# willow-ahrens/ChainPartitioners.jl

Hardware: AMD Instinct MI355X
Metric: partitions/sec, DynamicTotalSplitter(AffineConnectivityModel{Int64}(0,0,0,1)), K=64 (higher is better)
Workload: dtype int64; 1 GPU; config 3: DynamicTotalSplitter(AffineConnectivityModel{Int64}(0,0,0,1)) on suitesparse_shaped CSR (seeded SplitMix64 generator, tests/synth.py), n=10000000 rows, nnz=100000000, K=64; one independent partition per GPU; n=10000000, nnz=100000000, K=64, includes_oracle_build=True, device_block_pool=True

## Files before the change

chainpartitioners.jl_amd/csrc/capi.hip:

```cpp
#include "csr.hpp"
#include "model.hpp"
#include "dp.hpp"
#include "weight.hpp"
#include "sym.hpp"
#include "cut.hpp"
#include <cmath>
#include <memory>

using namespace cpk;

namespace cpk {

__global__ void __launch_bounds__(256) k_range_counts(int64_t nq, const int64_t *__restrict__ P, const int64_t *__restrict__ Rr,
                                                      const int64_t *__restrict__ pos, const int32_t *__restrict__ prev,
                                                      const int64_t *__restrict__ fpos, const int32_t *__restrict__ flast,
                                                      unsigned long long *__restrict__ nets, unsigned long long *__restrict__ selfnets)
{
    int64_t i = blockIdx.x;
    if (i >= nq) return;
    __shared__ int64_t sh[256];
    int64_t p = P[i], r = Rr[i];
    int64_t stride = (int64_t)gridDim.y * 256, start = (int64_t)blockIdx.y * 256 + threadIdx.x;
    int64_t c = 0;
    if (r > p) {
// ... 96 lines not shown

template <typename TC>
static int32_t oracle_eval_into(cp_csr_t A, const cp_model_t *model, const cp_rowpart_t *Pi, int64_t nq, const int64_t *j, const int64_t *jp,
                                const int64_t *k, TC *out)
{
    const bool i64 = std::is_same<TC, int64_t>::value;
    return cp_oracle_eval(A, model, Pi, CP_HINT_STEP, nq, j, jp, k, i64 ? (int64_t *)out : nullptr, i64 ? nullptr : (double *)out);
}

static const struct { const char *name; int64_t *var; bool kept; } g_stats[] = {
    {"spec_redo", &g_spec_redo, false}, {"poison_hits", &g_poison_hits, false}, {"fix_trips", &g_fix_trips, false},
    {"fix_edges", &g_fix_edges, false}, {"fix_items", &g_fix_items, false}, {"bn_sym_layers", &g_bn_sym_layers, true},
    {"own_split_tiles", &g_own_split_tiles, false}, {"gap_split_tiles", &g_gap_split_tiles, false},
    {"own_pair_waves", &g_own_pair_waves, false}, {"own_pair_lone", &g_own_pair_lone, false},
    {"overlap_isect", &g_overlap_isect, false}, {"cut_scan_layers", &g_cut_scan_layers, false},
};
static void stats_reset(bool all) { for (const auto &c : g_stats) if (all || !c.kept) *c.var = 0; }

enum OptRule { OPT_PLAIN, OPT_BOOL, OPT_CLAMP, OPT_POW2 };
constexpr int64_t NOLIM_LO = INT64_MIN, NOLIM_HI = INT64_MAX;
static const struct Opt { const char *name; int64_t *var; OptRule rule; int64_t lo, hi; } g_options[] = {
    {"force_brute", &g_opt_force_brute, OPT_PLAIN, 0, 0}, {"brute_max_n", &g_opt_brute_max_n, OPT_PLAIN, 0, 0}, {"dbg", &g_opt_dbg, OPT_PLAIN, 0, 0},
    {"short_t", &g_opt_short_t, OPT_PLAIN, 0, 0}, {"short_e", &g_opt_short_e, OPT_PLAIN, 0, 0}, {"ra_cache", &g_opt_ra_cache, OPT_PLAIN, 0, 0},
    {"leaf", &g_opt_leaf, OPT_PLAIN, 0, 0}, {"block_tables", &g_opt_block_tables, OPT_PLAIN, 0, 0}, {"nospec", &g_opt_nospec, OPT_PLAIN, 0, 0},
    {"rpass_small_tau", &g_opt_rpass_small_tau, OPT_PLAIN, 0, 0}, {"fixed_point", &g_opt_fixed_point, OPT_PLAIN, 0, 0},
    {"bn_wave", &g_opt_bn_wave, OPT_PLAIN, 0, 0},
    {"poison", &g_opt_poison, OPT_PLAIN, 0, 0},
    {"pool", &g_opt_pool, OPT_BOOL, 0, 0},
    {"own_blk", &g_opt_own_blk, OPT_BOOL, 0, 0},
    {"own_split", &g_opt_own_split, OPT_BOOL, 0, 0},
    {"own_pair", &g_opt_own_pair, OPT_BOOL, 0, 0},
    {"gap_split", &g_opt_gap_split, OPT_BOOL, 0, 0},
    {"lws", &g_opt_lws, OPT_BOOL, 0, 0},
    {"gap_tau", &g_opt_gap_tau, OPT_CLAMP, NOLIM_LO, 20}, {"gap_min", &g_opt_gap_min, OPT_CLAMP, 8, NOLIM_HI}, {"gap_nr", &g_opt_gap_nr, OPT_CLAMP, 1, 2},
    {"force_max", &g_opt_force_max, OPT_CLAMP, 0, NOLIM_HI}, {"rpass_cap", &g_opt_rpass_cap, OPT_CLAMP, 1, NOLIM_HI},
    {"own_min", &g_opt_own_min, OPT_CLAMP, 64, NOLIM_HI}, {"bn_chunk", &g_opt_bn_chunk, OPT_CLAMP, 1, NOLIM_HI},
    {"bn_slack", &g_opt_bn_slack, OPT_CLAMP, 0, NOLIM_HI}, {"bn_run", &g_opt_bn_run, OPT_CLAMP, 2, NOLIM_HI},
    {"rpass_ch", &g_opt_rpass_ch, OPT_POW2, 16, 4096}, {"setup_bs", &g_opt_setup_bs, OPT_POW2, 64, 1024}, {"lws_leaf", &g_opt_lws_leaf, OPT_POW2, 256, 2048},
};
static int64_t opt_value(const Opt &o, int64_t value)
{
    switch (o.rule) {
    case OPT_BOOL: return value ? 1 : 0;
    case OPT_CLAMP: return value < o.lo ? o.lo : value > o.hi ? o.hi : value;
    case OPT_POW2: { int64_t v = o.lo; while (v < value && v < o.hi) v <<= 1; return v; }
    default: return value;
    }
}

// ... 586 lines not shown
```

chainpartitioners.jl_amd/csrc/dp.hpp:

```cpp
#pragma once
#include "csr.hpp"
#include "model.hpp"

struct cp_dp_s {
    cp_csr_s *A = nullptr;
    int64_t K = 0;
    int32_t combine = 0, order = 0;
    bool fast = false, fast_bn = false, need_self = false;
    void *work = nullptr;
    cpk::DBuf<int32_t> ptr;
    int64_t rlo = 0, rhi = 0;
    int64_t wwin = 0;
    std::vector<int64_t> lay_lo, lay_hi;
    virtual ~cp_dp_s() = default;
    virtual int32_t step_layer(int64_t k, const void *cst_prev_device, void *cst_cur_device) = 0;
    virtual int32_t block_tables(int32_t *nplanes_out, int64_t *opt_out, int64_t *nets_out, int64_t *selfnets_out) = 0;
};

namespace cpk {

using DpBase = ::cp_dp_s;

struct DpWindow {
    int64_t w = 0;
// ... 84 lines not shown
extern int64_t g_opt_ra_cache;
extern int64_t g_opt_fixed_point;
extern int64_t g_opt_nospec;
extern int64_t g_spec_redo;
extern int64_t g_opt_rpass_small_tau;
extern int64_t g_opt_force_max;
extern int64_t g_opt_setup_bs;
extern int64_t g_opt_rpass_cap;
extern int64_t g_opt_rpass_ch;
extern int64_t g_opt_own_min;
extern int64_t g_opt_own_blk;
extern int64_t g_opt_own_split;
extern int64_t g_own_split_tiles;
extern int64_t g_opt_gap_split;
extern int64_t g_gap_split_tiles;
extern int64_t g_opt_own_pair;
extern int64_t g_own_pair_waves, g_own_pair_lone;
void dp_own_pair_test(int64_t nt, int64_t wave, int64_t *res);
extern int64_t g_overlap_isect;
void dp_own_split_test(cp_csr_s *A, int32_t *vpos_out, int32_t *vsa_out, int32_t *vnext_out, int64_t *res);
extern int64_t g_opt_short_t, g_opt_short_e;
extern int64_t g_opt_force_brute;
extern int64_t g_opt_brute_max_n;
extern int64_t g_opt_dbg;
enum DbgBit : int64_t {
    DBG_PRINT_ROUNDS = 8,
    DBG_NO_INTERIOR = 32,
    DBG_NO_OWN_TILES = 64,
    DBG_POISON = 128,
    DBG_POISON_ZERO = 256,
// ... 17 lines not shown
```

chainpartitioners.jl_amd/csrc/dp_brute.hip:

```cpp
#include "csr.hpp"
#include "model.hpp"
#include "dp.hpp"

namespace cpk {

int64_t g_opt_force_brute = 0;
int64_t g_opt_short_t = 8, g_opt_short_e = 64;
int64_t g_opt_own_min = 64;
int64_t g_opt_own_blk = 1;
int64_t g_opt_own_split = 1;
int64_t g_own_split_tiles = 0;
int64_t g_opt_gap_split = 1;
int64_t g_gap_split_tiles = 0;
int64_t g_opt_own_pair = 1;
int64_t g_own_pair_waves = 0, g_own_pair_lone = 0;
int64_t g_opt_rpass_ch = 256;
int64_t g_opt_rpass_small_tau = 4;
int64_t g_opt_force_max = 1024;
int64_t g_opt_setup_bs = 1024;
int64_t g_opt_rpass_cap = 200;
int64_t g_opt_nospec = 0, g_spec_redo = 0;
int64_t g_opt_gap_tau = 6, g_opt_gap_min = 64, g_opt_gap_nr = 2;
int64_t g_opt_ra_cache = 1;
int64_t g_opt_leaf = 1, g_opt_block_tables = 0;
int64_t g_opt_poison = 0, g_poison_hits = 0;
int64_t g_fix_trips = 0, g_fix_edges = 0, g_fix_items = 0;
int64_t g_opt_fixed_point = 0;
int64_t g_opt_brute_max_n = 200000;
int64_t g_opt_dbg = 0;

// ... 63 lines not shown
```

chainpartitioners.jl_amd/csrc/dp_total.hip:

```cpp
#include "dp_total.hpp"
#include <optional>

namespace cpk {

struct RoundDesc {
    int32_t isA, tau, nbits, nextra;
    Geo G;
    int64_t aoff[32];
    int64_t n, ntask;
    int64_t tbase[36];
    int64_t tskip[36];
    int64_t a_r0, a_nmain;
    int64_t extra[64];
    int32_t nlast, last_b[31];
    int32_t skip_std, skip_mir;
    int32_t fin_stamp;
};

__device__ __forceinline__ void decode_task(const RoundDesc &R, int64_t t, int64_t &r, int &b)
{
    if (R.G.win) {
        int bb = R.isA ? 0 : R.tau + 1;
        while (t >= R.tbase[bb + 1]) bb++;
        const int64_t l = t - R.tbase[bb] + R.tskip[bb];
// ... 1103 lines not shown
        for (int j = 0; j < 4; j++) {
            int32_t q = base + 64 * j + lane;
            fl[j] = false;
            if (q < e1) { int32_t v = arr[q]; fl[j] = GE ? (v >= thr) : (v < thr); }
        }
#pragma unroll
        for (int j = 0; j < 4; j++) {
            unsigned long long m = __ballot(fl[j]);
            int32_t w = myend - (base + 64 * j);
            if (w > 0) mine += __popcll(w >= 64 ? m : (m & ((1ull << w) - 1ull)));
        }
    }
    return c + mine;
}

template <typename TC, bool HYP>
struct GapCtx {
    const Best<TC, HYP> *part, *sub; const int32_t *spv; const uint8_t *spec;
    const int64_t *tilePS, *tilePS2;
    const int32_t *pos, *next, *fpos, *flast;
    const TC *W;
    int blk;
};

template <typename TC, bool HYP, int NR, bool SLOW>
__device__ __forceinline__ bool gap_walk(const GapCtx<TC, HYP> &C, const DevModel<TC> &M, TC alpha, int64_t ka, int64_t kz, int64_t k0,
                                         int32_t B, int32_t L, int32_t r, int32_t posr, const int32_t (&rr)[NR], const int32_t (&rcmp)[NR],
                                         const bool (&valid)[NR], int lane,
                                         TC (&bv)[NR], int32_t (&bp)[NR], int32_t (&bl)[NR], int32_t (&bl2)[NR], int32_t (&cum)[NR], int32_t (&cum2)[NR])
{
    const int64_t ps0 = C.tilePS[k0], ps20 = HYP ? C.tilePS2[k0] : 0;
    for (int64_t kb = ka; kb < kz; kb += 64) {
    const int64_t km = kb + lane < kz ? kb + lane : kz - 1;
    const int32_t m_base = (int32_t)(C.tilePS[km] - ps0), m_base2 = HYP ? (int32_t)(C.tilePS2[km] - ps20) : 0;
    const int m_ns = C.spec[km];
    Best<TC, HYP> m_part; best_clear(m_part);
    if (m_ns == 0) m_part = C.part[km];
    const int nb = (int)(kz - kb < 64 ? kz - kb : 64);
    Best<TC, HYP> nx_c; best_clear(nx_c);
    int32_t nx_sv = 0;
    {
        const int ns0 = rdl(m_ns, 0);
        if (ns0 > 0 && ns0 <= SMAX) { if (lane <= ns0) nx_c = C.sub[kb * (SMAX + 1) + lane]; if (lane < ns0) nx_sv = C.spv[kb * (SMAX + 1) + lane]; }
    }
    for (int i = 0; i < nb; i++) {
        const int64_t k = kb + i;
        const int32_t base = rdl(m_base, i), base2 = HYP ? rdl(m_base2, i) : 0;
        const int ns = rdl(m_ns, i);
        const Best<TC, HYP> cur_c = nx_c;
        const int32_t cur_sv = nx_sv;
        if (i + 1 < nb) {
            const int ns1 = rdl(m_ns, i + 1);
// ... 96 lines not shown
    g.rL = r - (1 << tau);
    int64_t hi64 = (int64_t)r + ((int64_t)1 << tau), re = ((((int64_t)r >> b) + 1) << b);
    if (hi64 > re) hi64 = re;
    if (hi64 > n + 1) hi64 = n + 1;
    g.hi = (int32_t)hi64;
    g.rr = g.rL + 1 + 64 * ck + lane;
    g.none = g.rL + 1 + 64 * ck >= g.hi;
    g.valid = g.rr < g.hi;
    g.rcmp = g.valid ? g.rr : INT32_MAX;
    return g;
}

template <typename TC, bool HYP>
struct GapSegRec { TC v; int32_t p, l, l2, cum, cum2, _pad; };

template <typename TC, bool HYP, int NR, bool SLOW>
__global__ void __launch_bounds__(256, 4) k_gap_finish(int tau, int nchunk, RoundCounts *__restrict__ rc, int64_t n,
                                                    const int64_t *__restrict__ toffs, GapCtx<TC, HYP> C,
                                                    const int4 *__restrict__ tdesc, const uint8_t *__restrict__ tb, const int32_t *__restrict__ rlen,
                                                    const int32_t *__restrict__ prev, const int32_t *__restrict__ lpos, const int32_t *__restrict__ lfirst,
                                                    DevModel<TC> M, TC alpha,
                                                    int32_t *__restrict__ opt, int32_t *__restrict__ nnopt, int32_t *__restrict__ nlopt, uint8_t *__restrict__ fin,
                                                    int2 *__restrict__ glist, int2 *__restrict__ gslot, int fin_stamp, int32_t *__restrict__ slow)
{
    const int lane = threadIdx.x & 63;
    const int nitem = (nchunk + NR - 1) / NR;
    const int64_t nwork = SLOW ? (int64_t)rc->n_gslow : (int64_t)rc->nown * nitem, n1 = n + 1;
    for (int64_t wi = (int64_t)blockIdx.x * 4 + (threadIdx.x >> 6); wi < nwork; wi += (int64_t)gridDim.x * 4) {
        const int64_t w = SLOW ? (int64_t)slow[wi] : wi;
        const int64_t t = w / nitem;
        const int ck0 = (int)(w - t * nitem) * NR;
        const int64_t k0 = toffs[t], k1 = toffs[t + 1];
        if (k1 - k0 > GAPSEG) {
            if (!SLOW && ck0 == 0 && lane == 0) {
                int nseg = (int)((k1 - k0 + GAPSEG - 1) / GAPSEG);
                int idx = atomicAdd(&rc->n_glong, 1), slot0 = atomicAdd(&rc->n_gslots, nseg);
                glist[idx] = make_int2((int)t, slot0);
                for (int j = 0; j < nseg; j++) gslot[slot0 + j] = make_int2((int)t, j);
            }
            continue;
        }
        const int4 td = tdesc[t];
// ... 6 lines not shown
        if (g[0].none) continue;
        int32_t Rr[NR], Rr2[NR];
#pragma unroll
        for (int u = 0; u < NR; u++) {
            Rr[u] = 0; Rr2[u] = 0;
            if (u == 0 || !g[u].none) {
                Rr[u] = gap_right_counts<false>(C.pos, prev, g[0].rL, ck0 + u, B, (int32_t)n, lane);
                if (HYP) Rr2[u] = gap_right_counts<true>(lpos, lfirst, g[0].rL, ck0 + u, B, (int32_t)n, lane);
            }
        }
        const int64_t rwL = (int64_t)b * n1 + prow(((int64_t)g[0].rL), n1 - 1);
        const int32_t anchor = nnopt[rwL], anchor2 = HYP ? nlopt[rwL] : 0;
        TC bv[NR]; int32_t bp[NR], bl[NR], bl2[NR], cum[NR], cum2[NR];
#pragma unroll
        for (int u = 0; u < NR; u++) { bv[u] = (TC)0; bp[u] = -1; bl[u] = 0; bl2[u] = 0; cum[u] = 0; cum2[u] = 0; }
        if (!gap_walk<TC, HYP, NR, SLOW>(C, M, alpha, k0, k1, k0, B, L, r, posr, rr, rcmp, valid, lane, bv, bp, bl, bl2, cum, cum2)) {
            if (lane == 0) slow[atomicAdd(&rc->n_gslow, 1)] = (int32_t)w;
            continue;
        }
#pragma unroll
        for (int u = 0; u < NR; u++) {
            if (valid[u]) {
                int64_t rw = (int64_t)b * n1 + prow(((int64_t)rr[u]), n1 - 1);
                opt[rw] = bp[u]; nnopt[rw] = anchor + Rr[u] + bl[u];
                if (HYP) nlopt[rw] = anchor2 + Rr2[u] + bl2[u];
                fin[rw] = (uint8_t)fin_stamp;
            }
        }
    }
}

// ... 6 lines not shown
    const int lane = threadIdx.x & 63;
    const int64_t nwork = SLOW ? (int64_t)rc->n_sslow : (int64_t)rc->n_gslots * nchunk;
    for (int64_t wi = (int64_t)blockIdx.x * 4 + (threadIdx.x >> 6); wi < nwork; wi += (int64_t)gridDim.x * 4) {
        const int64_t w = SLOW ? (int64_t)slow[wi] : wi;
        const int64_t slot = w / nchunk;
        const int ck = (int)(w - slot * nchunk);
        const int2 se = gslot[slot];
        const int64_t t = se.x, k0 = toffs[t], k1 = toffs[t + 1];
        const int sg = se.y;
        const int4 td = tdesc[t];
        const GapRows g = gap_rows(tau, ck, td.z, tb[t], n, lane);
        if (g.none) continue;
        TC bv[1] = {(TC)0}; int32_t bp[1] = {-1}, bl[1] = {0}, bl2[1] = {0}, cum[1] = {0}, cum2[1] = {0};
        const int32_t rr1[1] = {g.rr}, rcmp1[1] = {g.rcmp}; const bool valid1[1] = {g.valid};
        const int64_t ka = k0 + (int64_t)sg * GAPSEG, kz = ka + GAPSEG < k1 ? ka + GAPSEG : k1;
        if (!gap_walk<TC, HYP, 1, SLOW>(C, M, alpha, ka, kz, k0, td.x, rlen[t], td.z, td.w, rr1, rcmp1, valid1, lane, bv, bp, bl, bl2, cum, cum2)) {
            if (lane == 0) slow[atomicAdd(&rc->n_sslow, 1)] = (int32_t)w;
            continue;
        }
        GapSegRec<TC, HYP> rec; rec.v = bv[0]; rec.p = bp[0]; rec.l = bl[0]; rec.l2 = bl2[0]; rec.cum = cum[0]; rec.cum2 = cum2[0]; rec._pad = 0;
        gseg[(slot * nchunk + ck) * 64 + lane] = rec;
    }
}

template <typename TC, bool HYP>
__global__ void __launch_bounds__(256) k_gap_merge(int tau, int nchunk, const RoundCounts *__restrict__ rc, int64_t n, const int64_t *__restrict__ toffs,
                                                   const int4 *__restrict__ tdesc, const uint8_t *__restrict__ tb,
                                                   const int32_t *__restrict__ pos, const int32_t *__restrict__ prev, const int32_t *__restrict__ lpos,
                                                   const int32_t *__restrict__ lfirst, DevModel<TC> M, const int2 *__restrict__ glist,
                                                   const GapSegRec<TC, HYP> *__restrict__ gseg,
                                                   int32_t *__restrict__ opt, int32_t *__restrict__ nnopt, int32_t *__restrict__ nlopt, uint8_t *__restrict__ fin, int fin_stamp)
// ... 1367 lines not shown
    }
    Wk.win.built = true; Wk.win.w = w;
}

template <typename TC, bool HYP>
static void launch_gap(hipStream_t s, cp_csr_s *A, LayerWork<TC> &Wk, int tau, int nchunk, int gnr, RoundCounts *rc, int64_t n, const TC *W,
                       const DevModel<TC> &M, TC alpha, unsigned gg, unsigned gs_grid, unsigned gm, unsigned gslow_grid, int blk)
{
    GapCtx<TC, HYP> C{recs<HYP>(Wk.ow.o_part), recs<HYP>(Wk.ow.o_sub), Wk.ow.o_spv.p, Wk.ow.o_spec.p, Wk.ow.o_tilePS.p, if_hyp<HYP>(Wk.ow.o_tilePS2.p), A->pos32.p, A->next.p,
                      if_hyp<HYP>(A->fpos32.p), if_hyp<HYP>(A->flast.p), W, blk};
    auto *gs = reinterpret_cast<GapSegRec<TC, HYP> *>(Wk.gp.g_seg.p);
    const int32_t *lp = if_hyp<HYP>(A->lpos32.p), *lf = if_hyp<HYP>(A->lfirst.p);
    int32_t *nl = if_hyp<HYP>(Wk.pl.nlopt.p);
#define GF_ARGS tau, nchunk, rc, n, Wk.ow.o_toffs.p, C, Wk.ow.o_tdesc.p, Wk.ow.o_tb.p, Wk.ow.o_rlen.p, A->prev.p, lp, lf, M, alpha, Wk.pl.opt.p, Wk.pl.nnopt.p, nl, Wk.pl.fin.p, \
                Wk.gp.g_list.p, Wk.gp.g_slot.p, Wk.pl.fin_stamp, Wk.gp.g_slow.p
    if (gnr == 2) {
        hipLaunchKernelGGL(HIP_KERNEL_NAME(k_gap_finish<TC, HYP, 2, false>), dim3(gg), dim3(256), 0, s, GF_ARGS);
        hipLaunchKernelGGL(HIP_KERNEL_NAME(k_gap_finish<TC, HYP, 2, true>), dim3(gslow_grid), dim3(256), 0, s, GF_ARGS);
    } else {
        hipLaunchKernelGGL(HIP_KERNEL_NAME(k_gap_finish<TC, HYP, 1, false>), dim3(gg), dim3(256), 0, s, GF_ARGS);
        hipLaunchKernelGGL(HIP_KERNEL_NAME(k_gap_finish<TC, HYP, 1, true>), dim3(gslow_grid), dim3(256), 0, s, GF_ARGS);
    }
#undef GF_ARGS
#define GS_ARGS tau, nchunk, rc, n, Wk.ow.o_toffs.p, C, Wk.ow.o_tdesc.p, Wk.ow.o_tb.p, Wk.ow.o_rlen.p, M, alpha, Wk.gp.g_slot.p, gs, Wk.gp.g_sslow.p
    hipLaunchKernelGGL(HIP_KERNEL_NAME(k_gap_seg<TC, HYP, false>), dim3(gs_grid), dim3(256), 0, s, GS_ARGS);
    hipLaunchKernelGGL(HIP_KERNEL_NAME(k_gap_seg<TC, HYP, true>), dim3(gslow_grid), dim3(256), 0, s, GS_ARGS);
#undef GS_ARGS
    hipLaunchKernelGGL(HIP_KERNEL_NAME(k_gap_merge<TC, HYP>), dim3(gm), dim3(256), 0, s, tau, nchunk, rc, n, Wk.ow.o_toffs.p, Wk.ow.o_tdesc.p, Wk.ow.o_tb.p, A->pos32.p, A->prev.p,
                       lp, lf, M, Wk.gp.g_list.p, gs, Wk.pl.opt.p, Wk.pl.nnopt.p, nl, Wk.pl.fin.p, Wk.pl.fin_stamp);
}

constexpr int64_t LB_MAX = 1 << 20;

template <typename TC, bool HYP>
static void launch_round_a(const LayerCtx<TC> &C, LayerWork<TC> &Wk, const RaCache<TC> &Ra, const RATab &T, int64_t nrow_merge, int64_t tile0, int64_t tile1,
                           int bmin, bool mirrored, bool colmajor)
{
// ... 161 lines not shown
                       oblk ? Wk.ow.o_border.p : (const int32_t *)nullptr, A->pos32.p, A->next.p, if_hyp<HYP>(A->fpos32.p), if_hyp<HYP>(A->flast.p),
                       Wk.ow.o_tileS.p, Wk.ow.o_tileS2.p, Wk.ow.o_rec.p, Wk.ow.o_srec.p, C.W, C.M, C.alpha, recs<HYP>(Wk.ow.o_part), R.tau, Wk.ow.o_hi.p, Wk.ow.o_spec.p,
                       (int)((g_opt_dbg & DBG_GAP_ALL_SPECIAL) != 0), recs<HYP>(Wk.ow.o_sub), Wk.ow.o_spv.p, A->col.p, if_hyp<HYP>(A->ffirst.p),
                       split ? Wk.ow.split.vnext.p : (const int32_t *)nullptr, Wk.ow.split.vpos.p, Wk.ow.split.vsa.p, (int64_t)(n + 1));
}

template <typename TC, bool HYP>
static void own_merge(const LayerCtx<TC> &C, LayerWork<TC> &Wk, RoundCounts *rc, const RoundCounts &P)
{
    ProfScope ps(PROF_FIX, C.s, 24.0 * (double)P.NT);
    launch_fix_own<TC, HYP>(C.s, rc, Wk.ow.o_toffs.p, recs<HYP>(Wk.ow.o_part), Wk.ow.o_tdesc.p, Wk.ow.o_tb.p, if_hyp<HYP>(Wk.ow.o_tS0l.p), Wk.ow.o_tileS.p,
                            if_hyp<HYP>(Wk.ow.o_tileS2.p), C.M, Wk.pl.opt.p, Wk.pl.nnopt.p, if_hyp<HYP>(Wk.pl.nlopt.p), C.n, Wk.ow.o_items.p, Wk.ow.o_item_of.p, Wk.ow.o_trec.p,
                            Wk.ow.o_tick.p, C.spec ? grow_pred(P.NT) : P.NT, C.spec ? grow_pred(P.nown) : P.nown);
}

template <typename TC, bool HYP>
static void gap_finish(const LayerCtx<TC> &C, LayerWork<TC> &Wk, const RoundDesc &R, RoundCounts *rc, const RoundCounts &P)
{
    hipStream_t s = C.s;
    const int64_t gown = C.spec ? grow_pred(P.nown) : P.nown;
    {
        ProfScope ps(PROF_CARRY, s, 12.0 * (double)P.NT);
        const int32_t *ntp = reinterpret_cast<const int32_t *>(&rc->NT);
        exclusive_scan_i32_lb(Wk.ow.o_tileS.p, Wk.ow.o_tilePS.p, ntp, (int64_t)Wk.ow.o_tileS.n, nullptr, Wk.sc.scanws, s);
        if (HYP) exclusive_scan_i32_lb(Wk.ow.o_tileS2.p, Wk.ow.o_tilePS2.p, ntp, (int64_t)Wk.ow.o_tileS.n, nullptr, Wk.sc.scanws, s);
    }
    ProfScope ps(PROF_GAP, s, 24.0 * (double)P.NT);
    const int nchunk = (int)std::max<int64_t>(1, ((int64_t)2 << R.tau) / 64);
    const size_t ncap = Wk.ow.o_rec.n / GAPSEG + 2;
    Wk.gp.g_list.ensure(ncap); Wk.gp.g_slot.ensure(2 * ncap);
    Wk.gp.g_seg.ensure((2 * ncap) * (size_t)nchunk * 64 * sizeof(GapSegRec<TC, true>));
    Wk.gp.g_slow.ensure((size_t)gown * (size_t)nchunk + 64); Wk.gp.g_sslow.ensure((2 * ncap) * (size_t)nchunk + 64);
    CP_REQUIRE((int64_t)gown * nchunk < INT32_MAX && (int64_t)(2 * ncap) * nchunk < INT32_MAX, CP_EINTERNAL, "gap work index beyond 32 bits");
    const int gnr = (g_opt_gap_nr >= 2 && nchunk >= 2) ? 2 : 1;
    unsigned gg = (unsigned)std::min<int64_t>(cdiv(gown * cdiv((int64_t)nchunk, gnr), 4), 16384);
    unsigned gs_grid = (unsigned)std::min<int64_t>(cdiv((int64_t)(2 * ncap) * nchunk, 4), 8192);
    unsigned gm = (unsigned)std::min<int64_t>(cdiv((int64_t)ncap * nchunk, 4), 4096);
    const unsigned gslow_grid = 2048;
    launch_gap<TC, HYP>(s, C.A, Wk, R.tau, nchunk, gnr, rc, C.n, C.W, C.M, C.alpha, gg, gs_grid, gm, gslow_grid, C.oblk);
}

template <typename TC>
static int64_t flat_gtile(const LayerCtx<TC> &C, const LayerWork<TC> &Wk, const RoundCounts &P) { return C.spec ? (int64_t)Wk.fl.tileS.n : cdiv(P.T, LT); }

template <typename TC, bool HYP>
static void flat_stream(const LayerCtx<TC> &C, LayerWork<TC> &Wk, const RoundDesc &R, RoundCounts *rc, const RoundCounts &P)
{
    hipStream_t s = C.s;
    cp_csr_s *A = C.A;
    const int64_t gtile = flat_gtile(C, Wk, P);
// ... 91 lines not shown
    const int64_t n = C.n;
    const Geo G = C.G;
    const int nbits = C.nbits;
    int32_t *pzp = C.pzp;
    const int NR = nbits + 1;
    std::vector<RoundCounts> used((size_t)NR);
    memset(used.data(), 0, sizeof(RoundCounts) * (size_t)NR);
    struct Patch { size_t idx; int rd; int kind; int tau; bool split; };
    std::vector<Patch> patches;
    auto note = [&](int rd, int kind, int slot, int tau = 0, bool sp = false) {
        if (prof_active(slot)) patches.push_back({g_prof_pending.size() - 1, rd, kind, tau, sp});
    };
    bool any_forced = false;
    std::vector<int8_t> split_mode((size_t)NR, 0);
    std::vector<int8_t> pair_mode((size_t)NR, 0);

    for (int rd = 0; rd <= nbits; rd++) {
        RoundDesc R;
        if (rd == 0) make_round(R, true, 0, nbits, n, rlo, rhi, G, Wk.win.aoff);
        else make_round(R, false, nbits - rd, nbits, n, rlo, rhi, G, Wk.win.aoff);
        R.fin_stamp = Wk.pl.fin_stamp;
        if (C.leaf && !R.isA && R.tau < LEAF_T) continue;
        if (rd == 0 && g_opt_ra_cache && rlo <= 1 && rhi >= n && n >= 1 && !G.win) {
            round_a_full<TC, HYP>(C, Wk);
            R.a_nmain = 0; R.ntask = R.nextra + R.nlast;
        }
        if (rd == 0 && g_opt_ra_cache && G.win && G.s >= 1 && n >= 1 && !(g_opt_dbg & DBG_WIN_NO_RA_CACHE)) {
            std::optional<ProfScope> scope;
            round_a_win_std<TC, HYP>(C, Wk, scope);
            R.skip_std = 1;
// ... 23 lines not shown
        }
        round_scans<TC>(C, Wk, R, rc);
        if (!spec) {
            CP_HIP(hipMemcpyAsync(&P, rc, sizeof(P), hipMemcpyDeviceToHost, s));
            CP_HIP(hipStreamSynchronize(s));
            Wk.ow.ensure_own(Wk.hyp, (size_t)P.NT);
            Wk.fl.ensure_flat(Wk.hyp, (size_t)P.T);
        }
        used[(size_t)rd] = P;
        if (g_opt_dbg & DBG_PRINT_ROUNDS) fprintf(stderr, "round isA=%d tau=%d ntask=%lld %s long=%d own=%d T=%lld NT=%lld nontrivial=%d\n", R.isA, R.tau, (long long)R.ntask,
                                   spec ? "predicted" : "exact", P.nlong, P.nown, (long long)P.T, (long long)P.NT, P._pad);
        if (P.nown > 0 && P.NT > 0) {
            const int split = !(C.split_layer && !R.isA && (!gap || g_opt_gap_split)) ? 0 : R.tau + 1 >= SPLIT_BMIN ? 1 : 2;
            split_mode[(size_t)rd] = (int8_t)(gap ? -split : split);
            pair_mode[(size_t)rd] = own_pairs<HYP>(gap, G.win != 0);
            own_stream<TC, HYP>(C, Wk, R, rc, P, gap, split);
            note(rd, 0, gap ? PROF_GAPSTREAM : PROF_OWN, R.tau, split != 0);
            if (gap) gap_finish<TC, HYP>(C, Wk, R, rc, P);
            else own_merge<TC, HYP>(C, Wk, rc, P);
            CP_HIP(hipGetLastError());
        }
        if (P.nlong <= 0 || P.T <= 0) continue;
        flat_stream<TC, HYP>(C, Wk, R, rc, P);
        note(rd, 1, PROF_EXPAND);
        flat_finish<TC, HYP>(C, Wk, R, rc, P);
    }
    if (C.leaf) leaf_pass<TC, HYP>(C, Wk);
    combine_rows<TC, HYP>(C, Wk);
    CP_HIP(hipGetLastError());
    std::vector<RoundCounts> got((size_t)NR);
// ... 10 lines not shown
        if (g.nlong > 0 && g.T > 0 && !(u.nlong > 0 && u.T > 0)) ok = false;
    }
    if (pzp) {
        g_poison_hits += pz_hits[0];
        CP_REQUIRE(!(ok && pz_hits[0] > 0), CP_EINTERNAL, "a DP layer that is not redone read plane cells nobody wrote (poison mode)");
    }
    if (ok) Wk.ow.b_dirty = false;
    Wk.ow.t_dirty = false;
    if (ok) for (int rd = 0; rd < NR; rd++) { g_fix_trips += got[(size_t)rd].n_trips; g_fix_edges |= got[(size_t)rd].n_edge; }
    if (ok) for (int rd = 0; rd < NR; rd++) {
        const RoundCounts &g = got[(size_t)rd];
        if (g.nown > 0 && g.NT > 0) {
            const int sm = split_mode[(size_t)rd];
            (sm < 0 ? g_gap_split_tiles : g_own_split_tiles) += std::abs(sm) == 1 ? g.NT : std::abs(sm) == 2 ? g.n_split : 0;
            if (pair_mode[(size_t)rd]) { g_own_pair_waves += g.NT / 2; g_own_pair_lone += g.NT & 1; }
        }
    }
    for (int rd = 0; rd < NR; rd++) g_fix_items += got[(size_t)rd].n_items;
    if (ok) {
        for (auto &pt : patches) {
            const RoundCounts &g = got[(size_t)pt.rd];
            if (pt.idx < g_prof_pending.size())
                g_prof_pending[pt.idx].bytes = pt.kind == 0 ? C.own_bytes(Wk.ow.split, pt.tau, pt.split, (double)g.own_steps) : (double)g.T * C.step_bytes;
        }
        Wk.sp.pred = got; Wk.sp.pred_ok = true; Wk.sp.pred_rlo = rlo; Wk.sp.pred_rhi = rhi; Wk.sp.pred_win = G.win; Wk.sp.pred_w = G.w;
        if (allow_force && 2 * (rhi - rlo + 1) >= Wk.sp.force_rows) {
            Wk.sp.force_own.resize((size_t)NR, 0);
            Wk.sp.force_rows = rhi - rlo + 1;
            for (int rd = 1; rd < NR; rd++) {
                const RoundCounts &g = got[(size_t)rd];
// ... 24 lines not shown
        CP_HIP(hipMemsetAsync(Wk.pl.opt.p, 0, Wk.pl.opt.bytes(), A->stream));
        CP_HIP(hipMemsetAsync(Wk.pl.nnopt.p, 0, Wk.pl.nnopt.bytes(), A->stream));
        CP_HIP(hipMemsetAsync(Wk.pl.cr.p, 0, Wk.pl.cr.bytes(), A->stream));
        if (hyp) { CP_HIP(hipMemsetAsync(Wk.pl.nlopt.p, 0, Wk.pl.nlopt.bytes(), A->stream)); CP_HIP(hipMemsetAsync(Wk.pl.crl.p, 0, Wk.pl.crl.bytes(), A->stream)); }
        int64_t mx = n;
        for (int tau = 0; tau < nbits; tau++) { RoundDesc R; make_round(R, false, tau, nbits, n, 0, n); if (R.ntask > mx) mx = R.ntask; }
        for (int tau = 0; tau < nbits; tau++) mx = std::max<int64_t>(mx, ((n >> (tau + 1)) + 1) * (int64_t)(nbits - 1 - tau));
        mx = std::max<int64_t>(mx, 2 * n + nbits);
        Wk.max_tasks = mx > 0 ? mx : 1;
        size_t mt = (size_t)Wk.max_tasks;
        Wk.tk.tdesc.alloc(mt); Wk.tk.len.alloc(mt); Wk.tk.tb.alloc(mt); Wk.tk.offs.alloc(mt + 1);
        if (hyp) Wk.tk.tS0l.alloc(mt);
        int64_t mmin = std::max<int64_t>(2, std::min(g_opt_own_min, g_opt_gap_tau >= 0 ? g_opt_gap_min : g_opt_own_min));
        size_t mo = (size_t)(2 * n / mmin + 64) * (size_t)nbits + 1024;
        if (mo > mt) mo = mt;
        Wk.ow.o_tdesc.alloc(mo); Wk.ow.o_tb.alloc(mo); Wk.ow.o_rlen.alloc(mo); Wk.ow.o_ntl.alloc(mo); Wk.ow.o_toffs.alloc(mo + 1); Wk.ow.o_tick.alloc(mo);
        Wk.ow.t_dirty = true;
        if (hyp) Wk.ow.o_tS0l.alloc(mo);
        Wk.sp.rc.alloc((size_t)NBMAX + 2);
        Wk.pl.fin.alloc(plane); Wk.pl.last_s0.alloc(64); Wk.pl.fin_stamp = 255;
        Wk.n = n;
    }
    Geo G{0, 0, 0};
    if (wwin > 0) { G.win = 1; G.w = wwin; G.s = 0; while (((int64_t)2 << G.s) <= wwin) G.s++; if (G.s > nbits - 1) G.s = nbits - 1; }
    Wk.G = G;
    if (G.win && (!Wk.win.built || Wk.win.w != wwin)) win_build<TC>(A, Wk);
    bool spec = Wk.sp.pred_ok && !g_opt_nospec && Wk.sp.pred_win == G.win && Wk.sp.pred_w == G.w;
    Wk.sp.pred_scale = 1.0;
    if (spec && (Wk.sp.pred_rlo != rlo || Wk.sp.pred_rhi != rhi)) {
        const double a = (double)(Wk.sp.pred_rhi - Wk.sp.pred_rlo + 1), b = (double)(rhi - rlo + 1);
        if (!G.win || a < 1 || b < 1 || b > 2.0 * a) spec = false;
// ... 63 lines not shown
```

Baseline: 2.723 partitions/s.

## Add grouped gap-finish path with fused multi-row right counts and batched tile loads

Adds a GRP variant of k_gap_finish, on by default. It decodes work items with shifts instead of division and uses wave-uniform readfirstlane indices. Right counts for all NR rows come from one ballot/popcount pass over the column range instead of a separate count per row. Each short task's tile records are loaded once as a batch, and tasks longer than GAPSEG are deferred early. It also adds a tunable gap grid cap, stat counters, and pads the tb buffer to 4-byte alignment for word reads. The cost is larger kernels and more template instances, and the shift decode assumes nitem is a power of two.

```diff
diff --git a/chainpartitioners.jl_amd/csrc/capi.hip b/chainpartitioners.jl_amd/csrc/capi.hip
--- a/chainpartitioners.jl_amd/csrc/capi.hip
+++ b/chainpartitioners.jl_amd/csrc/capi.hip
@@ -134,6 +134,7 @@
     {"own_split_tiles", &g_own_split_tiles, false}, {"gap_split_tiles", &g_gap_split_tiles, false},
     {"own_pair_waves", &g_own_pair_waves, false}, {"own_pair_lone", &g_own_pair_lone, false},
     {"overlap_isect", &g_overlap_isect, false}, {"cut_scan_layers", &g_cut_scan_layers, false},
+    {"gap_fused_rc", &g_gap_fused_rc, false}, {"gap_long_tasks", &g_gap_long_tasks, false},
 };
 static void stats_reset(bool all) { for (const auto &c : g_stats) if (all || !c.kept) *c.var = 0; }
 
@@ -151,8 +152,10 @@
     {"own_split", &g_opt_own_split, OPT_BOOL, 0, 0},
     {"own_pair", &g_opt_own_pair, OPT_BOOL, 0, 0},
     {"gap_split", &g_opt_gap_split, OPT_BOOL, 0, 0},
+    {"gap_group", &g_opt_gap_group, OPT_BOOL, 0, 0},
     {"lws", &g_opt_lws, OPT_BOOL, 0, 0},
     {"gap_tau", &g_opt_gap_tau, OPT_CLAMP, NOLIM_LO, 20}, {"gap_min", &g_opt_gap_min, OPT_CLAMP, 8, NOLIM_HI}, {"gap_nr", &g_opt_gap_nr, OPT_CLAMP, 1, 2},
+    {"gap_grid", &g_opt_gap_grid, OPT_CLAMP, 1, 16384},
     {"force_max", &g_opt_force_max, OPT_CLAMP, 0, NOLIM_HI}, {"rpass_cap", &g_opt_rpass_cap, OPT_CLAMP, 1, NOLIM_HI},
     {"own_min", &g_opt_own_min, OPT_CLAMP, 64, NOLIM_HI}, {"bn_chunk", &g_opt_bn_chunk, OPT_CLAMP, 1, NOLIM_HI},
     {"bn_slack", &g_opt_bn_slack, OPT_CLAMP, 0, NOLIM_HI}, {"bn_run", &g_opt_bn_run, OPT_CLAMP, 2, NOLIM_HI},
diff --git a/chainpartitioners.jl_amd/csrc/dp.hpp b/chainpartitioners.jl_amd/csrc/dp.hpp
--- a/chainpartitioners.jl_amd/csrc/dp.hpp
+++ b/chainpartitioners.jl_amd/csrc/dp.hpp
@@ -122,6 +122,10 @@
 extern int64_t g_own_split_tiles;
 extern int64_t g_opt_gap_split;
 extern int64_t g_gap_split_tiles;
+extern int64_t g_opt_gap_group;
+extern int64_t g_gap_fused_rc;
+extern int64_t g_gap_long_tasks;
+extern int64_t g_opt_gap_grid;
 extern int64_t g_opt_own_pair;
 extern int64_t g_own_pair_waves, g_own_pair_lone;
 void dp_own_pair_test(int64_t nt, int64_t wave, int64_t *res);
diff --git a/chainpartitioners.jl_amd/csrc/dp_brute.hip b/chainpartitioners.jl_amd/csrc/dp_brute.hip
--- a/chainpartitioners.jl_amd/csrc/dp_brute.hip
+++ b/chainpartitioners.jl_amd/csrc/dp_brute.hip
@@ -14,6 +14,9 @@
 int64_t g_gap_split_tiles = 0;
 int64_t g_opt_own_pair = 1;
 int64_t g_own_pair_waves = 0, g_own_pair_lone = 0;
+int64_t g_opt_gap_group = 1;
+int64_t g_gap_fused_rc = 0, g_gap_long_tasks = 0;
+int64_t g_opt_gap_grid = 16384;
 int64_t g_opt_rpass_ch = 256;
 int64_t g_opt_rpass_small_tau = 4;
 int64_t g_opt_force_max = 1024;
diff --git a/chainpartitioners.jl_amd/csrc/dp_total.hip b/chainpartitioners.jl_amd/csrc/dp_total.hip
--- a/chainpartitioners.jl_amd/csrc/dp_total.hip
+++ b/chainpartitioners.jl_amd/csrc/dp_total.hip
@@ -1141,6 +1141,50 @@
     return c + mine;
 }
 
+template <int NR> struct GapCols { int32_t q0, e0, e1, myend[NR]; };
+template <int NR>
+__device__ __forceinline__ GapCols<NR> gap_cols(const int32_t *__restrict__ cpos, int32_t rL, int ck0, int nact, int32_t n, int lane)
+{
+    GapCols<NR> G;
+    int32_t cfirst = rL + 64 * ck0;
+    if (cfirst > n) cfirst = n;
+    int32_t cl = cfirst + 64 * nact;
+    if (cl > n) cl = n;
+    G.q0 = cpos[rL]; G.e0 = cpos[cfirst]; G.e1 = cpos[cl];
+#pragma unroll
+    for (int u = 0; u < NR; u++) {
+        int32_t jn = cfirst + 64 * u + lane + 1;
+        if (jn > cl) jn = cl;
+        G.myend[u] = cpos[jn];
+    }
+    return G;
+}
+template <bool GE, int NR>
+__device__ __forceinline__ void gap_right_counts_nr(const int32_t *__restrict__ arr, const GapCols<NR> &G, bool front, int32_t thr, int lane, int32_t (&out)[NR])
+{
+    int32_t c = 0;
+    if (front) {
+        for (int32_t q = G.q0 + lane; q < G.e0; q += 64) { int32_t v = arr[q]; c += GE ? (v >= thr) : (v < thr); }
+        for (int o = 32; o > 0; o >>= 1) c += __shfl_xor(c, o);
+    }
+#pragma unroll
+    for (int u = 0; u < NR; u++) out[u] = c;
+    for (int32_t base = G.e0; base < G.e1; base += 256) {
+        int32_t v[4];
+#pragma unroll
+        for (int j = 0; j < 4; j++) { int32_t q = base + 64 * j + lane; v[j] = arr[q < G.e1 ? q : G.e1 - 1]; }
+#pragma unroll
+        for (int j = 0; j < 4; j++) {
+            const unsigned long long m = __ballot((base + 64 * j + lane < G.e1) && (GE ? (v[j] >= thr) : (v[j] < thr)));
+#pragma unroll
+            for (int u = 0; u < NR; u++) {
+                const int32_t w = G.myend[u] - (base + 64 * j);
+                out[u] += __popcll(m & (w >= 64 ? ~0ull : w > 0 ? (1ull << w) - 1ull : 0ull));
+            }
+        }
+    }
+}
+
 template <typename TC, bool HYP>
 struct GapCtx {
     const Best<TC, HYP> *part, *sub; const int32_t *spv; const uint8_t *spec;
@@ -1150,19 +1194,36 @@
     int blk;
 };
 
-template <typename TC, bool HYP, int NR, bool SLOW>
+template <typename TC, bool HYP>
+struct GapBatch { int64_t ps, ps2; int m_ns; Best<TC, HYP> m_part; };
+template <typename TC, bool HYP>
+__device__ __forceinline__ GapBatch<TC, HYP> gap_batch(const GapCtx<TC, HYP> &C, int64_t kb, int64_t kz, int lane)
+{
+    GapBatch<TC, HYP> b;
+    const int64_t km = kb + lane < kz ? kb + lane : kz - 1;
+    b.ps = C.tilePS[km]; b.ps2 = HYP ? C.tilePS2[km] : 0;
+    b.m_ns = C.spec[km];
+    b.m_part = C.part[km];
+    return b;
+}
+
+static_assert(GAPSEG <= 64, "a GRP walk is one batch of tile records");
+template <typename TC, bool HYP, int NR, bool SLOW, bool GRP>
 __device__ __forceinline__ bool gap_walk(const GapCtx<TC, HYP> &C, const DevModel<TC> &M, TC alpha, int64_t ka, int64_t kz, int64_t k0,
                                          int32_t B, int32_t L, int32_t r, int32_t posr, const int32_t (&rr)[NR], const int32_t (&rcmp)[NR],
                                          const bool (&valid)[NR], int lane,
-                                         TC (&bv)[NR], int32_t (&bp)[NR], int32_t (&bl)[NR], int32_t (&bl2)[NR], int32_t (&cum)[NR], int32_t (&cum2)[NR])
-{
-    const int64_t ps0 = C.tilePS[k0], ps20 = HYP ? C.tilePS2[k0] : 0;
+                                         TC (&bv)[NR], int32_t (&bp)[NR], int32_t (&bl)[NR], int32_t (&bl2)[NR], int32_t (&cum)[NR], int32_t (&cum2)[NR],
+                                         const GapBatch<TC, HYP> &first, int64_t ps0g, int64_t ps20g)
+{
+    const int64_t ps0 = GRP ? ps0g : C.tilePS[k0], ps20 = GRP ? ps20g : HYP ? C.tilePS2[k0] : 0;
     for (int64_t kb = ka; kb < kz; kb += 64) {
+    if (GRP && kb != ka) break;
     const int64_t km = kb + lane < kz ? kb + lane : kz - 1;
-    const int32_t m_base = (int32_t)(C.tilePS[km] - ps0), m_base2 = HYP ? (int32_t)(C.tilePS2[km] - ps20) : 0;
-    const int m_ns = C.spec[km];
+    const int32_t m_base = (int32_t)((GRP ? first.ps : C.tilePS[km]) - ps0), m_base2 = HYP ? (int32_t)((GRP ? first.ps2 : C.tilePS2[km]) - ps20) : 0;
+    const int m_ns = GRP ? first.m_ns : C.spec[km];
     Best<TC, HYP> m_part; best_clear(m_part);
-    if (m_ns == 0) m_part = C.part[km];
+    if (GRP) m_part = first.m_part;
+    else if (m_ns == 0) m_part = C.part[km];
     const int nb = (int)(kz - kb < 64 ? kz - kb : 64);
     Best<TC, HYP> nx_c; best_clear(nx_c);
     int32_t nx_sv = 0;
@@ -1289,7 +1350,17 @@
 template <typename TC, bool HYP>
 struct GapSegRec { TC v; int32_t p, l, l2, cum, cum2, _pad; };
 
-template <typename TC, bool HYP, int NR, bool SLOW>
+struct GapHead { int64_t k0, k1; int4 td; int32_t L; int b; };
+__device__ __forceinline__ GapHead gap_head(const int64_t *__restrict__ toffs, const int4 *__restrict__ tdesc, const uint8_t *__restrict__ tb,
+                                            const int32_t *__restrict__ rlen, int64_t t)
+{
+    GapHead h;
+    h.k0 = toffs[t]; h.k1 = toffs[t + 1]; h.td = tdesc[t]; h.L = rlen[t];
+    h.b = (int)((reinterpret_cast<const uint32_t *>(tb)[t >> 2] >> (8 * (int)(t & 3))) & 255u);
+    return h;
+}
+
+template <typename TC, bool HYP, int NR, bool SLOW, bool GRP>
 __global__ void __launch_bounds__(256, 4) k_gap_finish(int tau, int nchunk, RoundCounts *__restrict__ rc, int64_t n,
                                                     const int64_t *__restrict__ toffs, GapCtx<TC, HYP> C,
                                                     const int4 *__restrict__ tdesc, const uint8_t *__restrict__ tb, const int32_t *__restrict__ rlen,
@@ -1301,6 +1372,65 @@
     const int lane = threadIdx.x & 63;
     const int nitem = (nchunk + NR - 1) / NR;
     const int64_t nwork = SLOW ? (int64_t)rc->n_gslow : (int64_t)rc->nown * nitem, n1 = n + 1;
+    if (GRP) {
+        const int ish = 31 - __clz(nitem);
+        for (int64_t wi = (int64_t)blockIdx.x * 4 + __builtin_amdgcn_readfirstlane((int)(threadIdx.x >> 6)); wi < nwork; wi += (int64_t)gridDim.x * 4) {
+            const int64_t w = SLOW ? (int64_t)__builtin_amdgcn_readfirstlane(slow[wi]) : wi;
+            const GapHead h = gap_head(toffs, tdesc, tb, rlen, w >> ish);
+            const int64_t t = w >> ish, k0 = h.k0, k1 = h.k1;
+            const int ck0 = (int)(w - (t << ish)) * NR;
+            if (k1 - k0 > GAPSEG) {
+                if (!SLOW && ck0 == 0 && lane == 0) {
+                    int nseg = (int)((k1 - k0 + GAPSEG - 1) / GAPSEG);
+                    int idx = atomicAdd(&rc->n_glong, 1), slot0 = atomicAdd(&rc->n_gslots, nseg);
+                    glist[idx] = make_int2((int)t, slot0);
+                    for (int j = 0; j < nseg; j++) gslot[slot0 + j] = make_int2((int)t, j);
+                }
+                continue;
+            }
+            const int b = h.b;
+            const int32_t B = h.td.x, r = h.td.z, posr = h.td.w, L = h.L;
+            GapRows g[NR];
+            int32_t rr[NR], rcmp[NR]; bool valid[NR];
+#pragma unroll
+            for (int u = 0; u < NR; u++) { g[u] = gap_rows(tau, ck0 + u, r, b, n, lane); rr[u] = g[u].rr; rcmp[u] = g[u].rcmp; valid[u] = g[u].valid; }
+            if (g[0].none) continue;
+            int nact = 1;
+#pragma unroll
+            for (int u = 1; u < NR; u++) nact += !g[u].none;
+            const GapCols<NR> gc = gap_cols<NR>(C.pos, g[0].rL, ck0, nact, (int32_t)n, lane);
+            GapCols<NR> gc2 = gc;
+            if (HYP) gc2 = gap_cols<NR>(lpos, g[0].rL, ck0, nact, (int32_t)n, lane);
+            const int64_t rwL = (int64_t)b * n1 + prow(((int64_t)g[0].rL), n1 - 1);
+            const int32_t anchor = nnopt[rwL], anchor2 = HYP ? nlopt[rwL] : 0;
+            const int64_t ps0 = C.tilePS[k0], ps20 = HYP ? C.tilePS2[k0] : 0;
+            const GapBatch<TC, HYP> gb = gap_batch<TC, HYP>(C, k0, k1, lane);
+            int32_t Rr[NR], Rr2[NR];
+            gap_right_counts_nr<false, NR>(prev, gc, ck0 > 0, B, lane, Rr);
+            if (HYP) gap_right_counts_nr<true, NR>(lfirst, gc2, ck0 > 0, B, lane, Rr2);
+            else {
+#pragma unroll
+                for (int u = 0; u < NR; u++) Rr2[u] = 0;
+            }
+            TC bv[NR]; int32_t bp[NR], bl[NR], bl2[NR], cum[NR], cum2[NR];
+#pragma unroll
+            for (int u = 0; u < NR; u++) { bv[u] = (TC)0; bp[u] = -1; bl[u] = 0; bl2[u] = 0; cum[u] = 0; cum2[u] = 0; }
+            if (!gap_walk<TC, HYP, NR, SLOW, true>(C, M, alpha, k0, k1, k0, B, L, r, posr, rr, rcmp, valid, lane, bv, bp, bl, bl2, cum, cum2, gb, ps0, ps20)) {
+                if (lane == 0) slow[atomicAdd(&rc->n_gslow, 1)] = (int32_t)w;
+                continue;
+            }
+#pragma unroll
+            for (int u = 0; u < NR; u++) {
+                if (valid[u]) {
+                    int64_t rw = (int64_t)b * n1 + prow(((int64_t)rr[u]), n1 - 1);
+                    opt[rw] = bp[u]; nnopt[rw] = anchor + Rr[u] + bl[u];
+                    if (HYP) nlopt[rw] = anchor2 + Rr2[u] + bl2[u];
+                    fin[rw] = (uint8_t)fin_stamp;
+                }
+            }
+        }
+        return;
+    }
     for (int64_t wi = (int64_t)blockIdx.x * 4 + (threadIdx.x >> 6); wi < nwork; wi += (int64_t)gridDim.x * 4) {
         const int64_t w = SLOW ? (int64_t)slow[wi] : wi;
         const int64_t t = w / nitem;
@@ -1337,7 +1467,7 @@
         TC bv[NR]; int32_t bp[NR], bl[NR], bl2[NR], cum[NR], cum2[NR];
 #pragma unroll
         for (int u = 0; u < NR; u++) { bv[u] = (TC)0; bp[u] = -1; bl[u] = 0; bl2[u] = 0; cum[u] = 0; cum2[u] = 0; }
-        if (!gap_walk<TC, HYP, NR, SLOW>(C, M, alpha, k0, k1, k0, B, L, r, posr, rr, rcmp, valid, lane, bv, bp, bl, bl2, cum, cum2)) {
+        if (!gap_walk<TC, HYP, NR, SLOW, false>(C, M, alpha, k0, k1, k0, B, L, r, posr, rr, rcmp, valid, lane, bv, bp, bl, bl2, cum, cum2, GapBatch<TC, HYP>(), 0, 0)) {
             if (lane == 0) slow[atomicAdd(&rc->n_gslow, 1)] = (int32_t)w;
             continue;
         }
@@ -1374,7 +1504,7 @@
         TC bv[1] = {(TC)0}; int32_t bp[1] = {-1}, bl[1] = {0}, bl2[1] = {0}, cum[1] = {0}, cum2[1] = {0};
         const int32_t rr1[1] = {g.rr}, rcmp1[1] = {g.rcmp}; const bool valid1[1] = {g.valid};
         const int64_t ka = k0 + (int64_t)sg * GAPSEG, kz = ka + GAPSEG < k1 ? ka + GAPSEG : k1;
-        if (!gap_walk<TC, HYP, 1, SLOW>(C, M, alpha, ka, kz, k0, td.x, rlen[t], td.z, td.w, rr1, rcmp1, valid1, lane, bv, bp, bl, bl2, cum, cum2)) {
+        if (!gap_walk<TC, HYP, 1, SLOW, false>(C, M, alpha, ka, kz, k0, td.x, rlen[t], td.z, td.w, rr1, rcmp1, valid1, lane, bv, bp, bl, bl2, cum, cum2, GapBatch<TC, HYP>(), 0, 0)) {
             if (lane == 0) slow[atomicAdd(&rc->n_sslow, 1)] = (int32_t)w;
             continue;
         }
@@ -2772,13 +2902,15 @@
     int32_t *nl = if_hyp<HYP>(Wk.pl.nlopt.p);
 #define GF_ARGS tau, nchunk, rc, n, Wk.ow.o_toffs.p, C, Wk.ow.o_tdesc.p, Wk.ow.o_tb.p, Wk.ow.o_rlen.p, A->prev.p, lp, lf, M, alpha, Wk.pl.opt.p, Wk.pl.nnopt.p, nl, Wk.pl.fin.p, \
                 Wk.gp.g_list.p, Wk.gp.g_slot.p, Wk.pl.fin_stamp, Wk.gp.g_slow.p
-    if (gnr == 2) {
-        hipLaunchKernelGGL(HIP_KERNEL_NAME(k_gap_finish<TC, HYP, 2, false>), dim3(gg), dim3(256), 0, s, GF_ARGS);
-        hipLaunchKernelGGL(HIP_KERNEL_NAME(k_gap_finish<TC, HYP, 2, true>), dim3(gslow_grid), dim3(256), 0, s, GF_ARGS);
-    } else {
-        hipLaunchKernelGGL(HIP_KERNEL_NAME(k_gap_finish<TC, HYP, 1, false>), dim3(gg), dim3(256), 0, s, GF_ARGS);
-        hipLaunchKernelGGL(HIP_KERNEL_NAME(k_gap_finish<TC, HYP, 1, true>), dim3(gslow_grid), dim3(256), 0, s, GF_ARGS);
-    }
+#define GF_PAIR(NR_, GRP_)                                                                                                              \
+    do {                                                                                                                            \
+        hipLaunchKernelGGL(HIP_KERNEL_NAME(k_gap_finish<TC, HYP, NR_, false, GRP_>), dim3(gg), dim3(256), 0, s, GF_ARGS);           \
+        hipLaunchKernelGGL(HIP_KERNEL_NAME(k_gap_finish<TC, HYP, NR_, true, GRP_>), dim3(gslow_grid), dim3(256), 0, s, GF_ARGS);    \
+    } while (0)
+    const bool grp = g_opt_gap_group != 0;
+    if (gnr == 2) { if (grp) GF_PAIR(2, true); else GF_PAIR(2, false); }
+    else { if (grp) GF_PAIR(1, true); else GF_PAIR(1, false); }
+#undef GF_PAIR
 #undef GF_ARGS
 #define GS_ARGS tau, nchunk, rc, n, Wk.ow.o_toffs.p, C, Wk.ow.o_tdesc.p, Wk.ow.o_tb.p, Wk.ow.o_rlen.p, M, alpha, Wk.gp.g_slot.p, gs, Wk.gp.g_sslow.p
     hipLaunchKernelGGL(HIP_KERNEL_NAME(k_gap_seg<TC, HYP, false>), dim3(gs_grid), dim3(256), 0, s, GS_ARGS);
@@ -2970,6 +3102,10 @@
                             Wk.ow.o_tick.p, C.spec ? grow_pred(P.NT) : P.NT, C.spec ? grow_pred(P.nown) : P.nown);
 }
 
+static int gap_nchunk(int tau) { return (int)std::max<int64_t>(1, ((int64_t)2 << tau) / 64); }
+static int gap_nr(int tau) { return (g_opt_gap_nr >= 2 && gap_nchunk(tau) >= 2) ? 2 : 1; }
+static int gap_fused_items(int tau) { return g_opt_gap_group != 0 && gap_nr(tau) == 2 ? gap_nchunk(tau) / 2 : 0; }
+
 template <typename TC, bool HYP>
 static void gap_finish(const LayerCtx<TC> &C, LayerWork<TC> &Wk, const RoundDesc &R, RoundCounts *rc, const RoundCounts &P)
 {
@@ -2982,14 +3118,14 @@
         if (HYP) exclusive_scan_i32_lb(Wk.ow.o_tileS2.p, Wk.ow.o_tilePS2.p, ntp, (int64_t)Wk.ow.o_tileS.n, nullptr, Wk.sc.scanws, s);
     }
     ProfScope ps(PROF_GAP, s, 24.0 * (double)P.NT);
-    const int nchunk = (int)std::max<int64_t>(1, ((int64_t)2 << R.tau) / 64);
+    const int nchunk = gap_nchunk(R.tau);
     const size_t ncap = Wk.ow.o_rec.n / GAPSEG + 2;
     Wk.gp.g_list.ensure(ncap); Wk.gp.g_slot.ensure(2 * ncap);
     Wk.gp.g_seg.ensure((2 * ncap) * (size_t)nchunk * 64 * sizeof(GapSegRec<TC, true>));
     Wk.gp.g_slow.ensure((size_t)gown * (size_t)nchunk + 64); Wk.gp.g_sslow.ensure((2 * ncap) * (size_t)nchunk + 64);
     CP_REQUIRE((int64_t)gown * nchunk < INT32_MAX && (int64_t)(2 * ncap) * nchunk < INT32_MAX, CP_EINTERNAL, "gap work index beyond 32 bits");
-    const int gnr = (g_opt_gap_nr >= 2 && nchunk >= 2) ? 2 : 1;
-    unsigned gg = (unsigned)std::min<int64_t>(cdiv(gown * cdiv((int64_t)nchunk, gnr), 4), 16384);
+    const int gnr = gap_nr(R.tau);
+    unsigned gg = (unsigned)std::min<int64_t>(cdiv(gown * cdiv((int64_t)nchunk, gnr), 4), g_opt_gap_grid);
     unsigned gs_grid = (unsigned)std::min<int64_t>(cdiv((int64_t)(2 * ncap) * nchunk, 4), 8192);
     unsigned gm = (unsigned)std::min<int64_t>(cdiv((int64_t)ncap * nchunk, 4), 4096);
     const unsigned gslow_grid = 2048;
@@ -3111,6 +3247,7 @@
     bool any_forced = false;
     std::vector<int8_t> split_mode((size_t)NR, 0);
     std::vector<int8_t> pair_mode((size_t)NR, 0);
+    std::vector<int32_t> fuse_items((size_t)NR, 0);
 
     for (int rd = 0; rd <= nbits; rd++) {
         RoundDesc R;
@@ -3164,6 +3301,7 @@
             const int split = !(C.split_layer && !R.isA && (!gap || g_opt_gap_split)) ? 0 : R.tau + 1 >= SPLIT_BMIN ? 1 : 2;
             split_mode[(size_t)rd] = (int8_t)(gap ? -split : split);
             pair_mode[(size_t)rd] = own_pairs<HYP>(gap, G.win != 0);
+            fuse_items[(size_t)rd] = gap ? gap_fused_items(R.tau) : 0;
             own_stream<TC, HYP>(C, Wk, R, rc, P, gap, split);
             note(rd, 0, gap ? PROF_GAPSTREAM : PROF_OWN, R.tau, split != 0);
             if (gap) gap_finish<TC, HYP>(C, Wk, R, rc, P);
@@ -3204,6 +3342,8 @@
             const int sm = split_mode[(size_t)rd];
             (sm < 0 ? g_gap_split_tiles : g_own_split_tiles) += std::abs(sm) == 1 ? g.NT : std::abs(sm) == 2 ? g.n_split : 0;
             if (pair_mode[(size_t)rd]) { g_own_pair_waves += g.NT / 2; g_own_pair_lone += g.NT & 1; }
+            g_gap_long_tasks += g.n_glong;
+            g_gap_fused_rc += (int64_t)(g.nown - g.n_glong) * fuse_items[(size_t)rd];
         }
     }
     for (int rd = 0; rd < NR; rd++) g_fix_items += got[(size_t)rd].n_items;
@@ -3258,7 +3398,7 @@
         int64_t mmin = std::max<int64_t>(2, std::min(g_opt_own_min, g_opt_gap_tau >= 0 ? g_opt_gap_min : g_opt_own_min));
         size_t mo = (size_t)(2 * n / mmin + 64) * (size_t)nbits + 1024;
         if (mo > mt) mo = mt;
-        Wk.ow.o_tdesc.alloc(mo); Wk.ow.o_tb.alloc(mo); Wk.ow.o_rlen.alloc(mo); Wk.ow.o_ntl.alloc(mo); Wk.ow.o_toffs.alloc(mo + 1); Wk.ow.o_tick.alloc(mo);
+        Wk.ow.o_tdesc.alloc(mo); Wk.ow.o_tb.alloc((mo + 3) & ~(size_t)3); Wk.ow.o_rlen.alloc(mo); Wk.ow.o_ntl.alloc(mo); Wk.ow.o_toffs.alloc(mo + 1); Wk.ow.o_tick.alloc(mo);
         Wk.ow.t_dirty = true;
         if (hyp) Wk.ow.o_tS0l.alloc(mo);
         Wk.sp.rc.alloc((size_t)NBMAX + 2);
```

Measured after the change: 2.779 partitions/s (median of 6 runs). +2.1%, better.
